# quenotl/PARESIS

Hardware: AMD Instinct MI355X
Metric: Mpixels/s, 4096^2 Fresnel+refraction step (higher is better)
Workload: dtype f32; 1 GPU; 4096x4096 fp32 study grid, 1 membrane position per GPU per step, 4 propagation distances z={1.6,3.6,5.2,7.2} m: 4 x (Fresnel propagation + refraction) from the 2-material membrane thickness maps (transmission evaluated inside the step); 52 keV, dSM/dMO/dOD=140/1.6/3.6 m; fresnel_engine=lds, streams=1, parallelism=single GPU

## Files before the change

include/paresis_hip.h:

```cpp
#ifndef PARESIS_HIP_H
#define PARESIS_HIP_H

#include <stddef.h>
#include <stdint.h>

#ifdef __cplusplus
extern "C" {
#endif

#define PSX_MAX_MAT 8
#define PSX_MAX_DIST 8
#define PSX_MAX_SRC 16

#define PSX_E_ARG (-1)
#define PSX_E_STATE (-2)
#define PSX_E_UNSUPPORTED (-3)

#define PSX_STATUS_NONFINITE 1u

typedef struct psx_fresnel_plan psx_fresnel_plan;
typedef struct psx_detector_plan psx_detector_plan;
typedef struct psx_integrate_plan psx_integrate_plan;

typedef struct { float re, im; } psx_c64;
// ... 54 lines not shown
int psx_fastloop_f32(const float *I, const float *Dx, const float *Dy, float *I2, int Nx, int Ny, void *stream);

#define PSX_ENGINE_AUTO 0
#define PSX_ENGINE_ROCFFT 1
#define PSX_ENGINE_LDS 2
int psx_fresnel_plan_create(int Nx, int Ny, int margin, int max_dist, int engine, psx_fresnel_plan **plan);
int psx_fresnel_plan_destroy(psx_fresnel_plan *plan);
int psx_fresnel_plan_engine(const psx_fresnel_plan *plan);
size_t psx_fresnel_plan_bytes(const psx_fresnel_plan *plan);
int psx_fresnel_plan_work_queue(psx_fresnel_plan *plan, int on);

int psx_fresnel_propagate(psx_fresnel_plan *plan, const psx_c64 *wave_in, float amp, const float *const *T,
                          const double *cphase, const double *catt, int nmat, int n_dist, const double *a,
                          const double *gphase, double du_x, double du_y, psx_c64 *const *wave_out,
                          float *const *inten_out, const float *inten_scale, int accumulate, void *stream);
int psx_fresnel_propagate_sources(psx_fresnel_plan *plan, int n_src, int n_dist, const psx_c64 *const *wave_in, const float *amp,
                                  const float *const *T, const double *cphase, const double *catt, int nmat, const double *a,
                                  const double *gphase, double du_x, double du_y, psx_c64 *const *wave_out,
                                  float *const *inten_out, const float *inten_scale, void *stream);

int psx_detector_plan_create(int Nx, int Ny, int ov, int nx, int ny, int margin, double sigma_src, double sigma_psf,
                             psx_detector_plan **plan);
int psx_detector_plan_destroy(psx_detector_plan *plan);
int psx_detect_f32(psx_detector_plan *plan, const float *img, float *out, void *stream);
#define PSX_MAX_DETECT 4
int psx_detect_multi_f32(psx_detector_plan *plan, const float *const *imgs, float *const *outs, int nimg, void *stream);
int psx_detector_operator_host(int N, int ov, int n, int margin, double sigma_src, double sigma_psf, int *start,
                               float *weights, int wcap, int *W_out);
int psx_resize_f32(const float *img, int Nx, int Ny, float *out, int sx, int sy, void *stream);
int psx_poisson_f32(const float *lam, float *out, int64_t n, uint64_t seed, void *stream);
// ... 72 lines not shown
```

paresis_amd/_lib.py:

```python
import ctypes
import os
from ctypes import POINTER, c_char_p, c_double, c_float, c_int, c_int64, c_size_t, c_uint64, c_void_p

_HERE = os.path.dirname(os.path.abspath(__file__))
LIB_PATH = os.path.join(_HERE, "libparesis_hip.so")

PSX_MAX_MAT = 8
PSX_MAX_FOLD = 64
PSX_MAX_LCS = 64
PSX_MAX_UMPA_WINDOW = 8
PSX_MAX_UMPA_SEARCH = 8
PSX_PHANTOM_TUBES = 12
PSX_MAX_DIST = 8
PSX_MAX_POISSON = 8
PSX_MAX_DETECT = 4
PSX_MAX_SRC = 16
PSX_SUM_SLOTS, PSX_SUM_STRIDE = 32, 16
ENGINE_AUTO, ENGINE_ROCFFT, ENGINE_LDS = 0, 1, 2
STATUS_NONFINITE = 1
ABI_VERSION = 14


class PsxError(RuntimeError):
    pass


_vp = c_void_p
_dp = POINTER(c_double)
_fp = POINTER(c_float)
_vpp = POINTER(c_void_p)

PROTOTYPES = {
    "psx_abi_version": (c_int, []),
    "psx_last_error": (c_char_p, []),
    "psx_device_ok": (c_int, []),
# ... 13 lines not shown
    "psx_refract_f32": (c_int, [_vp, c_float, _vpp, _dp, _dp, c_int, _vp, _vp, c_float, c_int, _vp, _vp, _vp, c_int,
                                c_int, c_int, c_double, c_double, c_double, _vp, _vp, _vp]),
    "psx_refract_split_f32": (c_int, [_vp, _vp, c_float, _vpp, _dp, _dp, c_int, _vp, _vp, _vp, c_float, c_int, c_int, c_int,
                                      c_int, c_double, c_double, c_double, _vp, _vp, _vp]),
    "psx_refract_multi_workspace_bytes": (c_size_t, [c_int, c_int, c_int]),
    "psx_refract_multi_f32": (c_int, [_vp, c_float, _vpp, _dp, _dp, c_int, _vp, _vpp, c_float, c_int, _vp, _vp, _vp,
                                      c_int, c_int, c_int, _dp, c_int, c_double, c_double, _vp, _vp, _vp]),
    "psx_refract_batch_workspace_bytes": (c_size_t, [c_int, c_int, c_int]),
    "psx_refract_batch_f32": (c_int, [c_int, _vpp, _fp, _vpp, _dp, _dp, c_int, _vpp, c_float, c_int, c_int, c_int, c_int, _dp,
                                      c_double, c_double, _vp, _vp, _vp]),
    "psx_fastloop_f32": (c_int, [_vp, _vp, _vp, _vp, c_int, c_int, _vp]),
    "psx_fresnel_plan_create": (c_int, [c_int, c_int, c_int, c_int, c_int, _vpp]),
    "psx_fresnel_plan_destroy": (c_int, [_vp]),
    "psx_fresnel_plan_engine": (c_int, [_vp]),
    "psx_fresnel_plan_bytes": (c_size_t, [_vp]),
    "psx_fresnel_plan_work_queue": (c_int, [_vp, c_int]),
    "psx_fresnel_propagate": (c_int, [_vp, _vp, c_float, _vpp, _dp, _dp, c_int, c_int, _dp, _dp, c_double, c_double,
                                      _vpp, _vpp, _fp, c_int, _vp]),
    "psx_fresnel_propagate_sources": (c_int, [_vp, c_int, c_int, _vpp, _fp, _vpp, _dp, _dp, c_int, _dp, _dp, c_double, c_double,
                                              _vpp, _vpp, _fp, _vp]),
    "psx_detector_plan_create": (c_int, [c_int, c_int, c_int, c_int, c_int, c_int, c_double, c_double, _vpp]),
    "psx_detector_plan_destroy": (c_int, [_vp]),
    "psx_detect_f32": (c_int, [_vp, _vp, _vp, _vp]),
    "psx_detect_multi_f32": (c_int, [_vp, _vpp, _vpp, c_int, _vp]),
    "psx_detector_operator_host": (c_int, [c_int, c_int, c_int, c_int, c_double, c_double, POINTER(c_int), _fp, c_int,
                                           POINTER(c_int)]),
    "psx_resize_f32": (c_int, [_vp, c_int, c_int, _vp, c_int, c_int, _vp]),
    "psx_poisson_f32": (c_int, [_vp, _vp, c_int64, c_uint64, _vp]),
    "psx_poisson_multi_f32": (c_int, [_vpp, POINTER(c_uint64), c_int, c_int64, _vp]),
    "psx_pack_counts_u16": (c_int, [_vp, _vp, c_int64, c_int64, _vp, _vp, c_int, _vp, _vp]),
# ... 62 lines not shown
```

paresis_amd/csrc/common.hpp:

```cpp
#pragma once
#include <hip/hip_runtime.h>

#include <atomic>
#include <cmath>
#include <cstdarg>
#include <cstdint>
#include <cstdio>
#include <memory>

#include "paresis_hip.h"

namespace psx {

char *err_buf();
int fail(int code, const char *fmt, ...);

#define PSX_HIP(expr)                                                                              \
    do {                                                                                           \
        hipError_t e__ = (expr);                                                                   \
        if (e__ != hipSuccess)                                                                     \
            return psx::fail((int)e__, "%s:%d: %s -> %s", __FILE__, __LINE__, #expr, hipGetErrorString(e__)); \
    } while (0)

#define PSX_REQUIRE(cond, ...)                         \
// ... 104 lines not shown
        case 0: { constexpr int NM = 0; __VA_ARGS__; } break; \
        case 1: { constexpr int NM = 1; __VA_ARGS__; } break; \
        case 2: { constexpr int NM = 2; __VA_ARGS__; } break; \
        case 3: { constexpr int NM = 3; __VA_ARGS__; } break; \
        case 4: { constexpr int NM = 4; __VA_ARGS__; } break; \
        default: { constexpr int NM = 8; __VA_ARGS__; } break; \
    }

extern unsigned long long *g_stamps;

enum DebugSwitch {
    DBG_STAMP_PASS1 = 0,
    DBG_STAMP_ROUND,
    DBG_DETECT_4PASS,
    DBG_NO_P2,
    DBG_COUNT
};
int debug_switch(DebugSwitch s);

bool prof_enabled();
int prof_begin(const char *name, hipStream_t st);
void prof_end(int handle, hipStream_t st);

struct ProfScope {
    int h;
    hipStream_t st;
    ProfScope(const char *name, hipStream_t s) : h(prof_enabled() ? prof_begin(name, s) : -1), st(s) {}
    ~ProfScope() {
        if (h >= 0) prof_end(h, st);
    }
// ... 32 lines not shown
```

paresis_amd/csrc/core.hip:

```cpp
#include <cstring>
#include <string>
#include <vector>

#include "common.hpp"

namespace psx {

char *err_buf() {
    static thread_local char buf[512] = "";
    return buf;
}

int fail(int code, const char *fmt, ...) {
    va_list ap;
    va_start(ap, fmt);
    vsnprintf(err_buf(), 512, fmt, ap);
    va_end(ap);
    return code;
}

int pack_mats(Mats &m, const float *const *T, const double *cphase, const double *catt, int nmat) {
    if (nmat < 0 || nmat > PSX_MAX_MAT) return fail(PSX_E_ARG, "nmat=%d outside [0,%d]", nmat, PSX_MAX_MAT);
    if (nmat > 0 && T == nullptr) return fail(PSX_E_ARG, "T is null with nmat=%d", nmat);
    m.n = nmat;
// ... 25 lines not shown
hipEvent_t take_event() {
    if (!g_pool.empty()) {
        hipEvent_t e = g_pool.back();
        g_pool.pop_back();
        return e;
    }
    hipEvent_t e = nullptr;
    (void)hipEventCreate(&e);
    return e;
}
}

unsigned long long *g_stamps = nullptr;

namespace {
const char *const g_dbg_names[DBG_COUNT] = {"stamp_pass1", "stamp_round", "detect_4pass", "no_p2"};
const int g_dbg_default[DBG_COUNT] = {0, 1, 0, 0};
std::atomic<int> g_dbg[DBG_COUNT] = {{0}, {1}, {0}, {0}};
}

int debug_switch(DebugSwitch s) { return g_dbg[s].load(std::memory_order_relaxed); }

bool prof_enabled() { return g_prof_on; }

int prof_begin(const char *name, hipStream_t st) {
    int id = -1;
    for (size_t i = 0; i < g_names.size(); ++i)
        if (g_names[i] == name) id = (int)i;
    if (id < 0) {
        g_names.push_back(name);
        id = (int)g_names.size() - 1;
    }
    ProfRec r{take_event(), take_event(), id};
// ... 13 lines not shown
    float acc = seed + threadIdx.x;
    while (wall_clock64() - r0 < ticks) {
#pragma unroll
        for (int i = 0; i < 64; ++i) acc = fmaf(acc, 1.0000001f, 0.5f);
    }
    const unsigned long long c1 = clock64(), r1 = wall_clock64();
    if (blockIdx.x == 0 && threadIdx.x == 0) {
        out[0] = c1 - c0;
        out[1] = r1 - r0;
    }
    if (acc == 12345.678f) out[2] = 1ull;
}

extern "C" {

int psx_abi_version(void) { return 14; }

const char *psx_last_error(void) { return psx::err_buf(); }

int psx_device_ok(void) {
    psx::DevBuf<int> d;
    int h = 0;
    if (d.alloc(1)) {
        psx::fail(1, "hipMalloc failed: no usable HIP device");
        return 0;
    }
    (void)hipMemset(d.get(), 0, sizeof(int));
    psx_probe_kernel<<<1, 1>>>(d.get());
    hipError_t e = hipGetLastError();
    if (e == hipSuccess) e = hipMemcpy(&h, d.get(), sizeof(int), hipMemcpyDeviceToHost);
    if (e != hipSuccess || h != 950) {
// ... 85 lines not shown
```

paresis_amd/csrc/fresnel.hip:

```cpp
#include "fresnel_plan.hpp"

using namespace psx;

namespace {

template <int NM>
__global__ __launch_bounds__(256) void k_pad_transmit(const float2 *__restrict__ wave_in, float amp, Mats m,
                                                      float2 *__restrict__ out, int Nx, int Ny, int margin, int Px,
                                                      int Py) {
    const int64_t n = (int64_t)Px * Py;
    for (int64_t q = (int64_t)blockIdx.x * blockDim.x + threadIdx.x; q < n; q += (int64_t)gridDim.x * blockDim.x) {
        const int pi = (int)(q / Py), pj = (int)(q - (int64_t)pi * Py);
        const int i = reflect_index(pi - margin, Nx), j = reflect_index(pj - margin, Ny);
        out[q] = source_wave<NM>(wave_in, amp, m, (int64_t)i * Ny + j);
    }
}

__global__ void k_chirp_table(float2 *table, int P, double a, double du, double sre, double sim) {
    const int i = blockIdx.x * blockDim.x + threadIdx.x;
    if (i >= P) return;
    const int f = (i < (P + 1) / 2) ? i : i - P;
    const double u = (double)f * du;
    const double ph = -a * u * u;
    const double r = ph - PSX_TWO_PI * rint(ph * PSX_INV_TWO_PI);
// ... 126 lines not shown
int psx_fresnel_plan_destroy(psx_fresnel_plan *p) {
    delete p;
    return 0;
}

int psx_fresnel_plan_engine(const psx_fresnel_plan *p) { return p ? p->engine : PSX_E_ARG; }

size_t psx_fresnel_plan_bytes(const psx_fresnel_plan *p) { return p ? p->bytes : 0; }

int psx_fresnel_plan_work_queue(psx_fresnel_plan *p, int on) {
    PSX_REQUIRE(p != nullptr, "psx_fresnel_plan_work_queue: null plan");
    if (p->engine == PSX_ENGINE_LDS) lds_engine_work_queue(p, on);
    return 0;
}

int psx_fresnel_propagate(psx_fresnel_plan *plan, const psx_c64 *wave_in, float amp, const float *const *T,
                          const double *cphase, const double *catt, int nmat, int n_dist, const double *a,
                          const double *gphase, double du_x, double du_y, psx_c64 *const *wave_out,
                          float *const *inten_out, const float *inten_scale, int accumulate, void *stream) {
    PSX_REQUIRE(plan != nullptr, "psx_fresnel_propagate: null plan");
    PSX_REQUIRE(n_dist >= 1 && n_dist <= plan->max_dist, "psx_fresnel_propagate: n_dist=%d outside [1,%d]", n_dist,
                plan->max_dist);
    PSX_REQUIRE(a != nullptr, "psx_fresnel_propagate: null distance table");
    PSX_REQUIRE(wave_out || inten_out, "psx_fresnel_propagate: no output requested");
    for (int d = 0; d < n_dist; ++d) {
        const bool w = wave_out && wave_out[d], i = inten_out && inten_out[d];
        PSX_REQUIRE(w || i, "psx_fresnel_propagate: distance %d has no output", d);
        PSX_REQUIRE(std::isfinite(a[d]), "psx_fresnel_propagate: a[%d] is not finite", d);
    }
    PropArgs pa;
// ... 36 lines not shown
```

paresis_amd/csrc/fresnel_lds.hip:

```cpp
#include <algorithm>
#include <cstdint>
#include <cstdlib>
#include <map>
#include <tuple>
#include <vector>

#include "fresnel_p2.hpp"
#include "fresnel_plan.hpp"
#include "fresnel_stages.hpp"

using namespace psx;
using namespace psx::lines;

namespace {

#define PSX_STAMP(k) PSX_STAMP_IF(k, tid == 0)
template <int R3, bool CONTIG, bool DUAL = false, bool QUEUE = false>
__global__ __launch_bounds__(T) void k_fresnel_lines(LineArgs a) {
    using GE = LineGeom<R3, false>;
    constexpr int M = GE::M, LINES = GE::LINES, S1 = GE::S1, MP = GE::MP;
    constexpr int LH = DUAL ? LINES / 2 : LINES;
    constexpr int LPG = LH;
    constexpr int LL = LH;
    static_assert(!DUAL || (CONTIG && LINES % 2 == 0), "DUAL: LINES/2 image lines x two distances per round");
// ... 1478 lines not shown
            }
            break;
        case Kind::P2: return p2::launch(t.radix, contig, dual, la, st, name);
        case Kind::P2X: return p2::x_launch(contig, la, st, name);
        case Kind::DIF: return contig ? launch_part<true, true>(la, st, name) : launch_part<false, true>(la, st, name);
        case Kind::PAIR: return contig ? launch_part<true, false>(la, st, name) : launch_part<false, false>(la, st, name);
    }
    return fail(PSX_E_UNSUPPORTED, "LDS engine: unsupported line length");
}

static int line_groups(const AxisTables &t, int nlines, bool dual) {
    const int lpg = t.kind == Kind::P2 ? p2::lines_per_round(t.radix, dual) : TOT / t.M / (dual ? 2 : 1);
    return (nlines + lpg - 1) / lpg;
}

static LineArgs pass_args(const psx_fresnel_plan *p, int pass, int n_dist) {
    const LdsEngine *e = p->lds.get();
    const AxisTables &t = e->ax[pass];
    LineArgs la;
    if (pass == 0) {
        la.N = p->Nx; la.nlines = p->Ny; la.P = p->Px;
        la.in_si = 1; la.in_sl = p->Nx; la.in_blocked = 0; la.out_ld = 0; la.out_blocked = 1;
    } else {
        la.N = p->Ny; la.nlines = p->Nx; la.P = p->Py;
        la.in_si = 0; la.in_sl = 0; la.in_blocked = 1; la.out_ld = p->Ny; la.out_blocked = 0;
    }
    la.margin = p->margin; la.L = la.N + la.P - 1;
    la.twA = t.twA.get(); la.twB = t.twB.get();
    la.B = t.B; la.Lh = t.Lh; la.S = t.S; la.NB = t.NB;
    la.w2 = t.w2.get(); la.w4 = t.w4.get(); la.wgpart = e->wgpart.get(); la.wg_groups = e->wgpart_groups;
    la.dsh = 2 * PART_M - la.P; la.thr = la.L - 2 * PART_M;
    la.queue = e->use_queue ? e->queue.get() + (size_t)pass * QUEUE_WORDS : nullptr;
    la.n_dist = n_dist; la.dist_inner = 0; la.accumulate = 0;
    la.stamps = nullptr; la.stamp_j = 1;
    return la;
}

int lds_engine_propagate(psx_fresnel_plan *p, const PropArgs &a) {
    LdsEngine *e = p->lds.get();
    hipStream_t st = a.stream;
    const int64_t npix = (int64_t)p->Nx * p->Ny;
    int nz[PSX_MAX_DIST], nnz = 0;
    for (int d = 0; d < a.n_dist; ++d) {
        if (a.a[d] != 0.0) {
            nz[nnz++] = d;
            continue;
        }
        PSX_DISPATCH_NMAT(a.m.n, PSX_TIMED("k_source_out", st, k_source_out<NM><<<ew_grid(npix, 256), 256, 0, st>>>(
                                                                   a.wave_in, a.amp, a.m, a.wave_out ? a.wave_out[d] : nullptr,
                                                                   a.inten_out ? a.inten_out[d] : nullptr,
                                                                   a.inten_scale ? a.inten_scale[d] : 1.f, a.accumulate,
                                                                   npix)));
    }
    if (nnz == 0) return launch_check("k_source_out");

    {
        const int ntiles = (int)(cdiv(p->Nx, 64) * cdiv(p->Ny, 64));
        int vec_ok = p->Ny % 4 == 0 && (uintptr_t)a.wave_in % 16 == 0;
        for (int i = 0; i < a.m.n && i < PSX_MAX_MAT; ++i) vec_ok = vec_ok && ((uintptr_t)a.m.T[i] % 16 == 0);
        PSX_DISPATCH_NMAT(a.m.n, PSX_TIMED("k_source_transposed", st, k_source_transposed<NM><<<ntiles, 256, 0, st>>>(
                                                                           a.wave_in, a.amp, a.m, e->pre.get(), p->Nx, p->Ny, vec_ok)));
        if (int rc = launch_check("k_source_transposed")) return rc;
    }

    const bool stamp_pass1 = debug_switch(DBG_STAMP_PASS1) != 0;
    const int stamp_round = debug_switch(DBG_STAMP_ROUND);
    {
        const AxisTables &t = e->ax[0];
        LineArgs la = pass_args(p, 0, nnz);
        la.stamps = stamp_pass1 ? g_stamps : nullptr; la.stamp_j = stamp_round;
        for (int i = 0; i < PSX_MAX_DIST; ++i) {
            const int k = i < nnz ? i : 0;
            la.src[i] = e->pre.get();
            if (i < nnz) {
                if (int rc = kernel_spectrum(p, e->ax[0], a.a[nz[i]], a.du_x, st, &la.H[i])) return rc;
            } else {
                la.H[i] = la.H[0];
            }
            la.wave_out[i] = e->inter.get() + (size_t)k * e->inter_elems;
            la.part[i] = la.wave_out[i];
            la.inten_out[i] = nullptr;
            la.scale[i] = 1.f;
            la.gph[i] = make_float2(1.f, 0.f);
        }
        const int cus = current_cu_count();
        switch (t.kind) {
            case Kind::R3:
            case Kind::P2: la.dist_inner = line_groups(t, p->Ny, nnz >= 2) >= cus; break;
            case Kind::DIF: la.dist_inner = nnz >= 2 && p->Ny >= cus; break;
            case Kind::P2X: la.dist_inner = p->Ny >= cus; break;
            case Kind::PAIR: break;
        }
        const bool dual = one_transform(t.kind) && la.dist_inner && nnz >= 2;
        if (dual && (nnz & 1)) {
            la.H[nnz] = la.H[nnz - 1];
            la.wave_out[nnz] = nullptr;
        }
        if (int rc = launch_axis(t, true, dual, la, st, "k_fresnel_cols")) return rc;
    }

    LineArgs lb = pass_args(p, 1, nnz);
    lb.accumulate = a.accumulate; lb.stamps = stamp_pass1 ? nullptr : g_stamps; lb.stamp_j = stamp_round;
    for (int i = 0; i < PSX_MAX_DIST; ++i) {
        const int k = i < nnz ? i : 0, d = nz[k];
        lb.src[i] = e->inter.get() + (size_t)k * e->inter_elems;
        if (i < nnz) {
            if (int rc = kernel_spectrum(p, e->ax[1], a.a[d], a.du_y, st, &lb.H[i])) return rc;
        } else {
            lb.H[i] = lb.H[0];
        }
        lb.wave_out[i] = a.wave_out ? a.wave_out[d] : nullptr;
        lb.part[i] = lb.wave_out[i] ? lb.wave_out[i] : (e->part ? e->part.get() + (size_t)k * npix : nullptr);
        lb.inten_out[i] = a.inten_out ? a.inten_out[d] : nullptr;
// ... 86 lines not shown
```

paresis_amd/csrc/fresnel_p2.hip:

```cpp
#include "fresnel_p2.hpp"

#include <atomic>

#include "fresnel_p2_dev.hpp"

using namespace psx;
using namespace psx::lines;
using namespace psx::p2dev;

namespace {

constexpr int TE = 512;
constexpr int TLD = 256;
constexpr int TT = TE + TLD;
constexpr int TOT2 = 16384;
constexpr int LXM = psx::p2::LXMAX;

template <int R1_, bool DUAL_>
struct G2 {
    static constexpr int R1 = R1_, M = 256 * R1, LINES = TOT2 / M, LH = DUAL_ ? LINES / 2 : LINES;
    static constexpr int MP = M + M / 32 + LXM;
    static constexpr int NBA = 32 / R1;
    static constexpr int SPL = M / 16;
    static constexpr int LB = R1 == 32 ? 5 : (R1 == 16 ? 4 : (R1 == 8 ? 3 : 2));
    static constexpr int LDP = LB | 1, LDB = 17;
    static constexpr int TPL = TLD / LINES, NCH = TPL >= 2 * LXM ? TPL / LXM : 1, CL = LXM / NCH;
    static constexpr int O_TP = LINES * MP, O_TB = O_TP + 256 * LDP, O_SA = O_TB + 16 * LDB, O_C = O_SA + LH * LXM,
                         O_UQ = O_C + NCH * LINES * LXM, O_HT = O_UQ + 2;
    static constexpr size_t lds_bytes(int ntap) { return sizeof(float2) * (size_t)(O_HT + ntap * LXM); }
    static constexpr int max_taps = (160 * 1024 / (int)sizeof(float2) - O_HT) / LXM < MAX_LINE ? (160 * 1024 / (int)sizeof(float2) - O_HT) / LXM : MAX_LINE;
    static_assert(LINES >= 2 && NBA >= 1 && max_taps >= 16, "LDS budget");
};

#define PSX_STAMP(k) PSX_STAMP_IF(k, tid == 0)

template <int R1, bool CONTIG, bool DUAL, bool QUEUE>
__global__ __launch_bounds__(TT) void k_fresnel_p2(LineArgs a) {
    using GE = G2<R1, DUAL>;
    constexpr int M = GE::M, LINES = GE::LINES, LH = GE::LH, MP = GE::MP, NBA = GE::NBA, SPL = GE::SPL, LDP = GE::LDP, LDB = GE::LDB;
    constexpr int NCH = GE::NCH, CL = GE::CL, TPL = GE::TPL;
    constexpr int LPG = LH;
    constexpr int LL = LH;
    static_assert(!DUAL || CONTIG, "DUAL is pass 1");
    extern __shared__ __attribute__((aligned(16))) float2 lds[];
    v2f *const Lb = reinterpret_cast<v2f *>(lds);
    v2f *const tP = Lb + GE::O_TP, *const tB = Lb + GE::O_TB;
    v2f *const SA = Lb + GE::O_SA;
    v2f *const CF = Lb + GE::O_C;
    v2f *const HT = Lb + GE::O_HT;
    int *const uq = reinterpret_cast<int *>(Lb + GE::O_UQ);
    const int tid = threadIdx.x;
    const int N = a.N, mg = a.margin;
    const int Lx = a.L - M;
    const bool upper_half = ((a.P - 1) >> 8) >= R1 / 2;

    const int ngroups = (a.nlines + LPG - 1) / LPG;
    const int nwork = a.dist_inner ? ngroups : ngroups * a.n_dist;
    const int xcd = blockIdx.x & 7, slot = blockIdx.x >> 3, nslot = gridDim.x >> 3;
    const int cq = nwork >> 3, cr = nwork & 7;
    const int cstart = xcd * cq + (xcd < cr ? xcd : cr), clen = cq + (xcd < cr ? 1 : 0);
    const int nunits = slot < clen ? (clen - slot + nslot - 1) / nslot : 0;
    const int nsub = DUAL ? (a.n_dist + 1) / 2 : a.n_dist;
    const int nj = a.dist_inner ? nunits * nsub : nunits;
    constexpr bool DYN = QUEUE;
    const int nsubr = a.dist_inner ? nsub : 1;
    auto item = [&](int j, int &d, int &g) __attribute__((always_inline)) {
        if (a.dist_inner) {
            const int u = j / nsub;
            d = j - u * nsub;
            g = cstart + (DYN ? uq[u & 3] : slot + u * nslot);
        } else {
            const int wk = cstart + (DYN ? uq[j & 3] : slot + j * nslot);
            d = wk / ngroups;
            g = wk - d * ngroups;
        }
    };
    auto valid = [&](int j) __attribute__((always_inline)) { return DYN ? uq[(j / nsubr) & 3] >= 0 : j < nj; };
    auto qcount = [&](int v) __attribute__((always_inline)) { return &a.queue[16 * (xcd + 8 * v)]; };
    auto share = [&](int v) __attribute__((always_inline)) { return v < clen ? (clen - v + nslot - 1) / nslot : 0; };
    bool dry = false, own_dry = false;
// ... 63 lines not shown
        const int ja = i0 + N + 2 * mg - 1, jb = i0 - 1;
        const int oa = phys(ja), ob = phys(jb);
        float2 *sa_line = lds + GE::O_SA + line * LXM;

        constexpr int CH = LL / 2 > 0 ? LL / 2 : 1, STEPV = TLD / CH, NLV = M / (2 * STEPV), PSTEPV = STEPV + STEPV / 32;
        static_assert(CONTIG || (LL % 2 == 0 && IB % 2 == 0 && STEPV % 32 == 0 && NLV * STEPV == M / 2), "16-byte loads of the blocked intermediate");
        const int c2 = lt % CH, i0v = lt / CH;
        float2 *base_v = lds + 2 * c2 * MP;
        const int jav = i0v + N + 2 * mg - 1, jbv = i0v - 1;
        const int oav = phys(jav), obv = phys(jbv);
        float2 *sa_v = lds + GE::O_SA + 2 * c2 * LXM;
        const int voff_v = ((((2 * c2) / IB) * N + i0v) * IB + (2 * c2) % IB) * (int)sizeof(float2);

        float2 xs[CONTIG ? NLD : 1], xm = make_float2(0.f, 0.f);
        float4 xv[CONTIG ? 1 : NLV];
        auto fetch = [&](int j) __attribute__((always_inline)) {
            int d, g;
            item(j, d, g);
            if (a.dist_inner && d != 0) return;
            const float2 *src = a.src[d];
            const int l0 = g * LPG;
            if constexpr (!CONTIG) {
                constexpr int LLB = LL > IB ? LL / IB : 1;
                const int nblk = min(LLB, (a.nlines - l0 + IB - 1) / IB);
                const __amdgpu_buffer_rsrc_t rs = __builtin_amdgcn_make_buffer_rsrc(
                    const_cast<float2 *>(src) + ((int64_t)(l0 / IB) * N) * IB + l0 % IB, 0,
                    nblk * N * IB * (int)sizeof(float2) - (l0 % IB) * (int)sizeof(float2), 0x00020000);
#pragma unroll
                for (int k = 0; k < NLV; ++k) {
                    const v4u r = __builtin_amdgcn_raw_buffer_load_b128(rs, voff_v + k * (STEPV * IB * (int)sizeof(float2)), 0, 0);
// ... 59 lines not shown
                    } else {
                        base[phys(ja + STEP * k)] = x;
                        if (k > 0 || jb >= 0) base[phys(jb + STEP * k)] = x;
                    }
                    if (STEP * k <= LXM) {
                        const int js = jb + STEP * k;
                        if ((unsigned)js < (unsigned)LXM) sa_line[js] = x;
                    }
                }
            }
            if (im >= 0) lds[lm * MP + phys(jm)] = l0 + lm < a.nlines ? xm : make_float2(0.f, 0.f);
            for (int t = lt + TLD; t < nmir; t += TLD) {
                const int ln = t % LL, r = t / LL;
                const int i2 = r < mg ? r + 1 : N - 1 - 2 * mg + r, j2 = r < mg ? N + 2 * mg - 1 - i2 : 2 * N - 3 - i2;
                float2 x2 = make_float2(0.f, 0.f);
                if (l0 + ln < a.nlines)
                    x2 = a.src[d][a.in_blocked ? ((int64_t)((l0 + ln) / IB) * N + i2) * IB + (l0 + ln) % IB
                                            : (int64_t)i2 * a.in_si + (int64_t)(l0 + ln) * a.in_sl];
                lds[ln * MP + phys(j2)] = x2;
            }
        };
        auto fixup = [&](int j) __attribute__((always_inline)) {
            if (Lx <= 0) return;
            int d, g;
            item(j, d, g);
            int lo = lt;
            asm volatile("" : "+v"(lo));
            const int lb = lo / TPL, r = lo % TPL;
            const int lbi = DUAL ? lb % LH : lb;
            const int dd = DUAL ? 2 * d + lb / LH : d;
            const v2f *ht = HT + dd * LXM;
            const v2f *sa = SA + lbi * LXM;
            const v2f *sb = Lb + lbi * MP + M + M / 32;
// ... 1 lines not shown
            for (int mp = NCH > 1 ? r % LXM : r; mp < LXM; mp += (NCH > 1 ? LXM : TPL)) {
                v2f acc = (v2f){0.f, 0.f};
#pragma unroll
                for (int tt = 0; tt < CL; ++tt) {
                    const int t = c * CL + tt;
                    const int jx = mp >= t ? mp - t : 0;
                    const v2f dl = lds_read(sb + jx) - lds_read(sa + jx);
                    const v2f term = pk_cmul(dl, lds_read(ht + t));
                    acc += mp >= t ? term : (v2f){0.f, 0.f};
                }
                CF[(c * LINES + lb) * LXM + mp] = acc;
            }
        };

        if (valid(0)) {
            fetch(0);
            spread(0);
        }
        lds_barrier();
        int ucur = 0, usub = 0;
        auto ring_ok = [&](int u) __attribute__((always_inline)) { return uq[u & 3] >= 0; };
        for (int j = 0; DYN ? ring_ok(ucur) : j < nj; ++j) {
            const bool last_sub = usub + 1 == nsubr;
            const bool more = DYN ? ring_ok(last_sub ? ucur + 1 : ucur) : j + 1 < nj;
            lds_barrier();
            if (a.stamps && lt == 0 && j == a.stamp_j) a.stamps[(size_t)blockIdx.x * 32 + 16] = wall_clock64();
            const bool qround = DYN && lt < 64 && usub == 0;
            const bool claiming = qround && ring_ok(ucur + 1);
            unsigned mine = 0xffffffffu;
            if (claiming && !own_dry && lt == 0) mine = atomicAdd(qcount(slot), 1u);
            if (more) fetch(j + 1);
            if (a.stamps && lt == 0 && j == a.stamp_j) a.stamps[(size_t)blockIdx.x * 32 + 17] = wall_clock64();
            fixup(j);
            lds_barrier();
            lds_barrier();
            if (a.stamps && lt == 0 && j == a.stamp_j) a.stamps[(size_t)blockIdx.x * 32 + 18] = wall_clock64();
            __builtin_amdgcn_s_setprio(3);
            if (more) spread(j + 1);
            __builtin_amdgcn_s_setprio(0);
            if (qround) {
                int unit = -1;
                if (claiming) {
                    const unsigned k = __builtin_amdgcn_readfirstlane(mine);
                    if (k < (unsigned)myshare) unit = slot + (int)k * nslot;
                    else own_dry = true;
                    if (unit < 0 && !dry) unit = steal();
                }
                if (lt == 0) uq[(ucur + 2) & 3] = unit;
// ... 223 lines not shown
                const int welems = lok ? (a.out_blocked ? ((N + IB - 1) / IB) * IB * a.nlines : N) : 0;
                if (upper_half)
                    store_legs<R1, R1 / 2>(v[i], v[i][0] + cf[i], wo, io, wbase, welems, e0, estep, (v2f){a.gph[dd].x, a.gph[dd].y},
                                           a.scale[dd], a.accumulate);
                else
                    store_legs<R1, 0>(v[i], v[i][0] + cf[i], wo, io, wbase, welems, e0, estep, (v2f){a.gph[dd].x, a.gph[dd].y},
                                      a.scale[dd], a.accumulate);
            }
        }
        PSX_STAMP(12);
        lds_barrier();
        PSX_STAMP(13);
    }
}

__global__ void k_p2_twiddles(float2 *twA, float2 *twB, int R1, int LB) {
    const int idx = blockIdx.x * blockDim.x + threadIdx.x;
    const int M = 256 * R1;
    if (idx < 256 * LB) {
        const int n = idx / LB, b = idx % LB;
        double s, c;
        sincospi(-2.0 * (double)((n << b) % M) / (double)M, &s, &c);
        twA[idx] = make_float2((float)c, (float)s);
    }
    if (idx < 256) {
        const int n = idx >> 4, k = idx & 15;
        double s, c;
        sincospi(-2.0 * (double)((n * k) % 256) / 256.0, &s, &c);
        twB[idx] = make_float2((float)c, (float)s);
    }
// ... 1 lines not shown

__global__ void k_p2_perm(const double2 *__restrict__ Hh, const double2 *__restrict__ hP, float2 *__restrict__ out, int R1, int P) {
    const int p = blockIdx.x * blockDim.x + threadIdx.x;
    const int M = 256 * R1;
    if (p < M) {
        const int k1 = p >> 8, k2 = (p >> 4) & 15, k3 = p & 15;
        const double2 v = Hh[k1 + R1 * k2 + 16 * R1 * k3];
        out[p] = make_float2((float)(v.x / M), (float)(v.y / M));
    } else if (p < M + LXM) {
        const int t = p - M;
        const double2 v = t < P ? hP[t] : make_double2(0.0, 0.0);
        out[p] = make_float2((float)(v.x / P), (float)(v.y / P));
    }
}

int line_grid_slots(int nwork, int cap) {
    int nslot = current_cu_count() / 8;
    if (nslot > (nwork + 7) / 8) nslot = (nwork + 7) / 8;
    if (cap && nslot > cap) nslot = cap;
    return nslot;
}

template <int R1, bool CONTIG, bool DUAL, bool QUEUE = false>
int launch_t(const LineArgs &la, hipStream_t st, const char *name) {
    if constexpr (!QUEUE) {
        if (la.queue) return launch_t<R1, CONTIG, DUAL, true>(la, st, name);
    }
    using GE = G2<R1, DUAL>;
    static std::atomic<unsigned long long> attr_mask{0};
    if (first_on_device(attr_mask))
        PSX_HIP(hipFuncSetAttribute((const void *)k_fresnel_p2<R1, CONTIG, DUAL, QUEUE>, hipFuncAttributeMaxDynamicSharedMemorySize,
                                    (int)GE::lds_bytes(GE::max_taps)));
    if (la.n_dist < 1 || la.n_dist > MAX_LINE || (DUAL && !la.dist_inner))
        return fail(PSX_E_STATE, "LDS engine (power-of-two lines): %d distances, dist_inner %d", la.n_dist, la.dist_inner);
    const int ntap = DUAL ? 2 * ((la.n_dist + 1) / 2) : la.n_dist;
    if (ntap > GE::max_taps) return fail(PSX_E_STATE, "LDS engine (power-of-two lines): %d distances in one launch, %d fit", ntap, GE::max_taps);
    const int nwork = ((la.nlines + GE::LH - 1) / GE::LH) * (la.dist_inner ? 1 : la.n_dist);
    const int nslot = line_grid_slots(nwork, QUEUE ? 32 : 0);
    PSX_TIMED(name, st, k_fresnel_p2<R1, CONTIG, DUAL, QUEUE><<<8 * nslot, TT, GE::lds_bytes(ntap), st>>>(la));
    const int rc = launch_check(name);
    if constexpr (QUEUE) {
        if (rc) (void)hipMemsetAsync(la.queue, 0, sizeof(unsigned) * QUEUE_WORDS, st);
    }
    return rc;
}

template <int R1>
int launch_r(bool contig, bool dual, const LineArgs &la, hipStream_t st, const char *name) {
    if (dual) return launch_t<R1, true, true>(la, st, name);
    return contig ? launch_t<R1, true, false>(la, st, name) : launch_t<R1, false, false>(la, st, name);
}

}

namespace psx {
namespace p2 {

int pick_r1(int N, int margin) {
    const int P = N + 2 * margin, L = N + P - 1;
    for (int r1 : {4, 8, 16, 32}) {
        const int M = 256 * r1;
        if (N <= M / 2 && P <= M && L - M <= LXMAX && L - M <= N - 1) return r1;
    }
    return 0;
}

static int log2_r1(int R1) { return R1 == 32 ? 5 : (R1 == 16 ? 4 : (R1 == 8 ? 3 : 2)); }
size_t twA_elems(int R1) { return (size_t)256 * log2_r1(R1); }
int max_distances(int R1) {
    switch (R1) {
        case 4: return G2<4, false>::max_taps;
// ... 15 lines not shown
    const int n = 256 * R1 + LXMAX;
    PSX_TIMED("k_kern_perm", st, k_p2_perm<<<(n + 255) / 256, 256, 0, st>>>(Hh, hP, out, R1, P));
    return launch_check("k_p2_perm");
}

int launch(int R1, bool contig, bool dual, const lines::LineArgs &la, hipStream_t st, const char *name) {
    switch (R1) {
        case 4: return launch_r<4>(contig, dual, la, st, name);
        case 8: return launch_r<8>(contig, dual, la, st, name);
        case 16: return launch_r<16>(contig, dual, la, st, name);
        case 32: return launch_r<32>(contig, dual, la, st, name);
    }
    return fail(PSX_E_UNSUPPORTED, "LDS engine (power-of-two lines): unsupported radix %d", R1);
}

}
}
```

paresis_amd/csrc/fresnel_p2.hpp:

```cpp
#pragma once
#include "fresnel_stages.hpp"

namespace psx {
namespace p2 {

constexpr int LXMAX = 32;

int pick_r1(int N, int margin);

size_t twA_elems(int R1);
size_t twB_elems();
int build_tables(float2 *twA, float2 *twB, int R1, hipStream_t st);

size_t spectrum_elems(int R1);
int perm_spectrum(const double2 *Hh, const double2 *hP, float2 *out, int R1, int P, hipStream_t st);

int launch(int R1, bool contig, bool dual, const lines::LineArgs &la, hipStream_t st, const char *name);

int max_distances(int R1);

int lines_per_round(int R1, bool dual);

bool x_serves(int N, int margin);
int x_points();
size_t x_spectrum_elems();
size_t x_line_buffer_elems();
int x_build_twiddles(float2 *w2, float2 *w4, hipStream_t st);
int x_pad_taps(const double2 *hP, double2 *buf, int P, hipStream_t st);
int x_perm_spectrum(const double2 *Hh, const double2 *hP, float2 *out, int P, hipStream_t st);
int x_launch(bool contig, const lines::LineArgs &la, hipStream_t st, const char *name);

}
}
// ... 1 lines not shown
```

paresis_amd/csrc/fresnel_plan.hpp:

```cpp
#pragma once
#include <rocfft/rocfft.h>

#include "common.hpp"

#define PSX_ROCFFT(expr)                                                                          \
    do {                                                                                          \
        rocfft_status s__ = (expr);                                                               \
        if (s__ != rocfft_status_success)                                                         \
            return psx::fail(1000 + (int)s__, "%s:%d: %s -> rocfft_status %d", __FILE__, __LINE__, #expr, (int)s__); \
    } while (0)

namespace psx {

int rocfft_ensure_setup();

class FftPlan {
    rocfft_plan plan_[2] = {nullptr, nullptr};
    rocfft_execution_info info_ = nullptr;
    DevBuf<char> work_;

  public:
    enum Dir { FWD = 0, INV = 1, BOTH = 2 };
    FftPlan() = default;
    FftPlan(const FftPlan &) = delete;
// ... 97 lines not shown
    pa.du_x = a.du_x; pa.du_y = a.du_y;
    pa.wave_out = a.wave_out ? a.wave_out + (size_t)s * a.n_dist : nullptr;
    pa.inten_out = a.inten_out ? a.inten_out + (size_t)s * a.n_dist : nullptr;
    pa.inten_scale = a.inten_scale ? a.inten_scale + (size_t)s * a.n_dist : nullptr;
    pa.accumulate = 0; pa.stream = a.stream;
    return pa;
}

int rocfft_engine_create(psx_fresnel_plan *p);
int rocfft_engine_propagate(psx_fresnel_plan *p, const PropArgs &a);

bool lds_engine_supported(int Nx, int Ny, int margin);
int lds_engine_create(psx_fresnel_plan *p);
int lds_engine_propagate(psx_fresnel_plan *p, const PropArgs &a);
void lds_engine_work_queue(psx_fresnel_plan *p, int on);
int lds_engine_propagate_sources(psx_fresnel_plan *p, const SourcesArgs &a);

template <int NM>
__device__ __forceinline__ float2 source_wave(const float2 *__restrict__ wave_in, float amp, const Mats &m, int64_t p) {
    float2 w = wave_in ? wave_in[p] : make_float2(1.f, 0.f);
    float a = amp;
    if (NM > 0) {
        double ph, la;
        mats_eval<NM>(m, p, ph, la);
        float c, s;
        cis_f64(ph, c, s);
        a *= exp_att(la);
        w = make_float2(w.x * c - w.y * s, w.x * s + w.y * c);
    }
    return make_float2(a * w.x, a * w.y);
}

__host__ __device__ __forceinline__ int reflect_index(int q, int n) {
    if (q < 0) q = -q;
    if (q >= n) q = 2 * (n - 1) - q;
    return q;
}

}
```

paresis_amd/csrc/fresnel_stages.hpp:

```cpp
#pragma once
#include <cstdint>
#include <type_traits>

#include "fft_pk.hpp"
#include "common.hpp"

namespace psx {
namespace lines {

typedef unsigned v2u __attribute__((ext_vector_type(2)));
typedef unsigned v4u __attribute__((ext_vector_type(4)));

constexpr int TC = 768;
constexpr int TL = 256;
constexpr int T = TC + TL;
constexpr int TOT = 18432;
constexpr int RAD = 24;
constexpr int IB = 8;
constexpr int IBS = 3;
static_assert((1 << IBS) == IB, "intermediate block size");
constexpr int SAMPLE_SHIFT = 3;
constexpr int BLOCKED_SAMPLE_SHIFT = IBS + SAMPLE_SHIFT;
static_assert((1 << SAMPLE_SHIFT) == sizeof(float2) && (1 << BLOCKED_SAMPLE_SHIFT) == IB * sizeof(float2),
              "sample strides of the intermediate");
// ... 16 lines not shown
    int out_blocked;
    const float2 *twA, *twB;
    const float2 *H[MAX_LINE];
    float2 *wave_out[MAX_LINE];
    float *inten_out[MAX_LINE];
    float scale[MAX_LINE];
    float2 gph[MAX_LINE];
    int accumulate;
    int B, Lh, S, NB;
    float2 *part[MAX_LINE];
    const float2 *w2;
    const float2 *w4;
    float2 *wgpart;
    int wg_groups;
    int dsh, thr;
    unsigned *queue;
    unsigned long long *stamps;
    int stamp_j;
};

#define PSX_STAMP_IF(k, who)                                                                       \
    do {                                                                                           \
        if (a.stamps && j == a.stamp_j && (who)) a.stamps[(size_t)blockIdx.x * 32 + (k)] = wall_clock64(); \
    } while (0)

__device__ __forceinline__ void wave_sync() {
    __builtin_amdgcn_fence(__ATOMIC_RELEASE, "wavefront");
    __builtin_amdgcn_wave_barrier();
    __builtin_amdgcn_fence(__ATOMIC_ACQUIRE, "wavefront");
}
// ... 204 lines not shown
```

Baseline: 62530 Mpixel/s.

## Fuse source-wave evaluation from thickness maps into the first LDS Fresnel pass

Adds a fused-source variant of the power-of-two LDS column kernel. It reads the material thickness maps directly through buffer loads and evaluates the transmitted wave in registers, instead of first writing a precomputed source field to an intermediate buffer and reading it back. This removes one full-grid complex write and read per step. The cost is extra register pressure and double-precision cis/exp work inside the FFT kernel, along with more template instantiations and a separate translation unit. It is gated on radix, map count, no wave input and no work queue, and can be disabled with a debug switch.

Result: slower. 54840 Mpixel/s (-12.3%).

```diff
diff --git a/include/paresis_hip.h b/include/paresis_hip.h
--- a/include/paresis_hip.h
+++ b/include/paresis_hip.h
@@ -92,6 +92,7 @@
                           const double *cphase, const double *catt, int nmat, int n_dist, const double *a,
                           const double *gphase, double du_x, double du_y, psx_c64 *const *wave_out,
                           float *const *inten_out, const float *inten_scale, int accumulate, void *stream);
+int psx_fresnel_fused_source(int Nx, int Ny, int margin, int n_dist, int nmat, int has_wave_in);
 int psx_fresnel_propagate_sources(psx_fresnel_plan *plan, int n_src, int n_dist, const psx_c64 *const *wave_in, const float *amp,
                                   const float *const *T, const double *cphase, const double *catt, int nmat, const double *a,
                                   const double *gphase, double du_x, double du_y, psx_c64 *const *wave_out,
diff --git a/paresis_amd/_lib.py b/paresis_amd/_lib.py
--- a/paresis_amd/_lib.py
+++ b/paresis_amd/_lib.py
@@ -18,7 +18,7 @@
 PSX_SUM_SLOTS, PSX_SUM_STRIDE = 32, 16
 ENGINE_AUTO, ENGINE_ROCFFT, ENGINE_LDS = 0, 1, 2
 STATUS_NONFINITE = 1
-ABI_VERSION = 14
+ABI_VERSION = 15
 
 
 class PsxError(RuntimeError):
@@ -62,6 +62,7 @@
     "psx_fresnel_plan_destroy": (c_int, [_vp]),
     "psx_fresnel_plan_engine": (c_int, [_vp]),
     "psx_fresnel_plan_bytes": (c_size_t, [_vp]),
+    "psx_fresnel_fused_source": (c_int, [c_int, c_int, c_int, c_int, c_int, c_int]),
     "psx_fresnel_plan_work_queue": (c_int, [_vp, c_int]),
     "psx_fresnel_propagate": (c_int, [_vp, _vp, c_float, _vpp, _dp, _dp, c_int, c_int, _dp, _dp, c_double, c_double,
                                       _vpp, _vpp, _fp, c_int, _vp]),
diff --git a/paresis_amd/csrc/common.hpp b/paresis_amd/csrc/common.hpp
--- a/paresis_amd/csrc/common.hpp
+++ b/paresis_amd/csrc/common.hpp
@@ -142,6 +142,7 @@
     DBG_STAMP_ROUND,
     DBG_DETECT_4PASS,
     DBG_NO_P2,
+    DBG_NO_FUSED_SOURCE,
     DBG_COUNT
 };
 int debug_switch(DebugSwitch s);
diff --git a/paresis_amd/csrc/core.hip b/paresis_amd/csrc/core.hip
--- a/paresis_amd/csrc/core.hip
+++ b/paresis_amd/csrc/core.hip
@@ -63,9 +63,9 @@
 unsigned long long *g_stamps = nullptr;
 
 namespace {
-const char *const g_dbg_names[DBG_COUNT] = {"stamp_pass1", "stamp_round", "detect_4pass", "no_p2"};
-const int g_dbg_default[DBG_COUNT] = {0, 1, 0, 0};
-std::atomic<int> g_dbg[DBG_COUNT] = {{0}, {1}, {0}, {0}};
+const char *const g_dbg_names[DBG_COUNT] = {"stamp_pass1", "stamp_round", "detect_4pass", "no_p2", "no_fused_source"};
+const int g_dbg_default[DBG_COUNT] = {0, 1, 0, 0, 0};
+std::atomic<int> g_dbg[DBG_COUNT] = {{0}, {1}, {0}, {0}, {0}};
 }
 
 int debug_switch(DebugSwitch s) { return g_dbg[s].load(std::memory_order_relaxed); }
@@ -109,7 +109,7 @@
 
 extern "C" {
 
-int psx_abi_version(void) { return 14; }
+int psx_abi_version(void) { return 15; }
 
 const char *psx_last_error(void) { return psx::err_buf(); }
 
diff --git a/paresis_amd/csrc/fresnel.hip b/paresis_amd/csrc/fresnel.hip
--- a/paresis_amd/csrc/fresnel.hip
+++ b/paresis_amd/csrc/fresnel.hip
@@ -164,6 +164,12 @@
     return 0;
 }
 
+int psx_fresnel_fused_source(int Nx, int Ny, int margin, int n_dist, int nmat, int has_wave_in) {
+    PSX_REQUIRE(Nx >= 2 && Ny >= 2 && margin >= 0 && margin < Nx && margin < Ny, "psx_fresnel_fused_source: grid %dx%d, margin %d", Nx, Ny, margin);
+    PSX_REQUIRE(n_dist >= 0 && n_dist <= PSX_MAX_DIST && nmat >= 0, "psx_fresnel_fused_source: %d distances, %d maps", n_dist, nmat);
+    return lds_engine_fused_source(Nx, Ny, margin, n_dist, nmat, has_wave_in != 0) ? 1 : 0;
+}
+
 int psx_fresnel_propagate(psx_fresnel_plan *plan, const psx_c64 *wave_in, float amp, const float *const *T,
                           const double *cphase, const double *catt, int nmat, int n_dist, const double *a,
                           const double *gphase, double du_x, double du_y, psx_c64 *const *wave_out,
diff --git a/paresis_amd/csrc/fresnel_lds.hip b/paresis_amd/csrc/fresnel_lds.hip
--- a/paresis_amd/csrc/fresnel_lds.hip
+++ b/paresis_amd/csrc/fresnel_lds.hip
@@ -1516,6 +1516,16 @@
     return (nlines + lpg - 1) / lpg;
 }
 
+static bool fused_source_rule(const AxisKind &t, int Nx, int Ny, int nnz, int nmat, bool wave_in, bool queue) {
+    if (t.kind != Kind::P2 || nnz < 1) return false;
+    return p2::fused_source_serves(t.radix, Nx, Ny, nmat, wave_in, queue);
+}
+
+bool lds_engine_fused_source(int Nx, int Ny, int margin, int n_dist, int nmat, bool wave_in) {
+    if (!lds_engine_supported(Nx, Ny, margin)) return false;
+    return fused_source_rule(choose(Nx, margin), Nx, Ny, n_dist, nmat, wave_in, false);
+}
+
 static LineArgs pass_args(const psx_fresnel_plan *p, int pass, int n_dist) {
     const LdsEngine *e = p->lds.get();
     const AxisTables &t = e->ax[pass];
@@ -1534,6 +1544,7 @@
     la.dsh = 2 * PART_M - la.P; la.thr = la.L - 2 * PART_M;
     la.queue = e->use_queue ? e->queue.get() + (size_t)pass * QUEUE_WORDS : nullptr;
     la.n_dist = n_dist; la.dist_inner = 0; la.accumulate = 0;
+    la.mats = Mats{}; la.amp = 0.f; la.src_ny = 0;
     la.stamps = nullptr; la.stamp_j = 1;
     return la;
 }
@@ -1556,7 +1567,9 @@
     }
     if (nnz == 0) return launch_check("k_source_out");
 
-    {
+    const bool fused = debug_switch(DBG_NO_FUSED_SOURCE) == 0 &&
+                       fused_source_rule(e->ax[0], p->Nx, p->Ny, nnz, a.m.n, a.wave_in != nullptr, e->use_queue);
+    if (!fused) {
         const int ntiles = (int)(cdiv(p->Nx, 64) * cdiv(p->Ny, 64));
         int vec_ok = p->Ny % 4 == 0 && (uintptr_t)a.wave_in % 16 == 0;
         for (int i = 0; i < a.m.n && i < PSX_MAX_MAT; ++i) vec_ok = vec_ok && ((uintptr_t)a.m.T[i] % 16 == 0);
@@ -1573,7 +1586,7 @@
         la.stamps = stamp_pass1 ? g_stamps : nullptr; la.stamp_j = stamp_round;
         for (int i = 0; i < PSX_MAX_DIST; ++i) {
             const int k = i < nnz ? i : 0;
-            la.src[i] = e->pre.get();
+            la.src[i] = fused ? nullptr : e->pre.get();
             if (i < nnz) {
                 if (int rc = kernel_spectrum(p, e->ax[0], a.a[nz[i]], a.du_x, st, &la.H[i])) return rc;
             } else {
@@ -1598,7 +1611,14 @@
             la.H[nnz] = la.H[nnz - 1];
             la.wave_out[nnz] = nullptr;
         }
-        if (int rc = launch_axis(t, true, dual, la, st, "k_fresnel_cols")) return rc;
+        if (fused) {
+            la.mats = a.m; la.amp = a.amp; la.src_ny = p->Ny;
+            if (la.L - t.M > p2::LXMAX || la.N != t.N)
+                return fail(PSX_E_UNSUPPORTED, "LDS engine: a line of %d samples (%d points) on an axis built for %d", la.N, la.L, t.N);
+            if (int rc = p2::launch_fused(t.radix, dual, la, st, "k_fresnel_cols")) return rc;
+        } else if (int rc = launch_axis(t, true, dual, la, st, "k_fresnel_cols")) {
+            return rc;
+        }
     }
 
     LineArgs lb = pass_args(p, 1, nnz);
diff --git a/paresis_amd/csrc/fresnel_p2.hip b/paresis_amd/csrc/fresnel_p2.hip
--- a/paresis_amd/csrc/fresnel_p2.hip
+++ b/paresis_amd/csrc/fresnel_p2.hip
@@ -3,6 +3,11 @@
 #include <atomic>
 
 #include "fresnel_p2_dev.hpp"
+#include "fresnel_plan.hpp"
+
+#ifndef PSX_P2_FUSED_TU
+#define PSX_P2_FUSED_TU 0
+#endif
 
 using namespace psx;
 using namespace psx::lines;
@@ -34,8 +39,10 @@
 
 #define PSX_STAMP(k) PSX_STAMP_IF(k, tid == 0)
 
-template <int R1, bool CONTIG, bool DUAL, bool QUEUE>
+template <int R1, bool CONTIG, bool DUAL, bool QUEUE, int SRC = 0>
 __global__ __launch_bounds__(TT) void k_fresnel_p2(LineArgs a) {
+    static_assert(SRC == 0 || (CONTIG && !QUEUE && SRC <= (R1 == 4 ? 3 : 4)), "fused source: pass 1, static shares, at most four maps (R1 = 4: three)");
+    constexpr bool FUSED = SRC > 0;
     using GE = G2<R1, DUAL>;
     constexpr int M = GE::M, LINES = GE::LINES, LH = GE::LH, MP = GE::MP, NBA = GE::NBA, SPL = GE::SPL, LDP = GE::LDP, LDB = GE::LDB;
     constexpr int NCH = GE::NCH, CL = GE::CL, TPL = GE::TPL;
@@ -63,7 +70,8 @@
     const int nsub = DUAL ? (a.n_dist + 1) / 2 : a.n_dist;
     const int nj = a.dist_inner ? nunits * nsub : nunits;
     constexpr bool DYN = QUEUE;
-    const int nsubr = a.dist_inner ? nsub : 1;
+    constexpr bool FUSED1 = FUSED && !DUAL;
+    const int nsubr = FUSED1 ? 1 : (a.dist_inner ? nsub : 1);
     auto item = [&](int j, int &d, int &g) __attribute__((always_inline)) {
         if (a.dist_inner) {
             const int u = j / nsub;
@@ -157,6 +165,51 @@
 
         float2 xs[CONTIG ? NLD : 1], xm = make_float2(0.f, 0.f);
         float4 xv[CONTIG ? 1 : NLV];
+        constexpr int NM = FUSED ? SRC : 1;
+        constexpr int NPART = FUSED && !DUAL && NM * NLD > 96 ? 2 : 1, KPART = NLD / NPART;
+        float tr[FUSED ? KPART : 1][NM], tm[NM];
+        using KAll = std::integral_constant<int, FUSED ? NLD : 0>;
+        using KNone = std::integral_constant<int, 0>;
+        auto gather = [&](int j, auto k0c, auto k1c) __attribute__((always_inline)) {
+            constexpr int K0 = decltype(k0c)::value, K1 = decltype(k1c)::value;
+            int d, g;
+            item(j, d, g);
+            const int l0 = g * LPG;
+            const int voff = (i0 * a.src_ny + l0 + line) * (int)sizeof(float), vstep = STEP * a.src_ny * (int)sizeof(float);
+            const int voffm = (im >= 0 && l0 + lm < a.nlines) ? (im * a.src_ny + l0 + lm) * (int)sizeof(float) : 0;
+            __amdgpu_buffer_rsrc_t rs[NM];
+#pragma unroll
+            for (int m = 0; m < NM; ++m)
+                rs[m] = __builtin_amdgcn_make_buffer_rsrc(const_cast<float *>(a.mats.T[m]), 0, N * a.src_ny * (int)sizeof(float), 0x00020000);
+#pragma unroll
+            for (int k = K0; k < K1; ++k) {
+#pragma unroll
+                for (int m = 0; m < NM; ++m)
+                    tr[k - K0][m] = __builtin_bit_cast(float, __builtin_amdgcn_raw_buffer_load_b32(rs[m], voff + k * vstep, 0, 0));
+            }
+            if constexpr (K0 == 0) {
+#pragma unroll
+                for (int m = 0; m < NM; ++m) tm[m] = __builtin_bit_cast(float, __builtin_amdgcn_raw_buffer_load_b32(rs[m], voffm, 0, 0));
+            }
+        };
+        auto evaluate = [&](auto k0c, auto k1c) __attribute__((always_inline)) {
+            constexpr int K0 = decltype(k0c)::value, K1 = decltype(k1c)::value;
+#pragma unroll
+            for (int k = K0; k < K1; ++k) {
+                xs[k] = source_wave_maps<NM>(a.amp, a.mats, tr[k - K0]);
+                if (k % 4 == 3) __builtin_amdgcn_sched_barrier(0);
+            }
+            if constexpr (K0 == 0) xm = source_wave_maps<NM>(a.amp, a.mats, tm);
+        };
+        auto gather_evaluate = [&](int j) __attribute__((always_inline)) {
+            auto part = [&](auto pc) __attribute__((always_inline)) {
+                constexpr int K0 = decltype(pc)::value * KPART;
+                gather(j, std::integral_constant<int, K0>{}, std::integral_constant<int, K0 + KPART>{});
+                evaluate(std::integral_constant<int, K0>{}, std::integral_constant<int, K0 + KPART>{});
+            };
+            part(std::integral_constant<int, 0>{});
+            if constexpr (NPART == 2) part(std::integral_constant<int, 1>{});
+        };
         auto fetch = [&](int j) __attribute__((always_inline)) {
             int d, g;
             item(j, d, g);
@@ -246,9 +299,19 @@
                 const int ln = t % LL, r = t / LL;
                 const int i2 = r < mg ? r + 1 : N - 1 - 2 * mg + r, j2 = r < mg ? N + 2 * mg - 1 - i2 : 2 * N - 3 - i2;
                 float2 x2 = make_float2(0.f, 0.f);
-                if (l0 + ln < a.nlines)
-                    x2 = a.src[d][a.in_blocked ? ((int64_t)((l0 + ln) / IB) * N + i2) * IB + (l0 + ln) % IB
-                                            : (int64_t)i2 * a.in_si + (int64_t)(l0 + ln) * a.in_sl];
+                if (l0 + ln < a.nlines) {
+                    if constexpr (FUSED) {
+                        float t2[NM];
+#pragma unroll
+                        for (int m = 0; m < NM; ++m)
+                            t2[m] = __builtin_bit_cast(float, __builtin_amdgcn_raw_buffer_load_b32(
+                                __builtin_amdgcn_make_buffer_rsrc(const_cast<float *>(a.mats.T[m]), 0, N * a.src_ny * (int)sizeof(float), 0x00020000),
+                                (i2 * a.src_ny + l0 + ln) * (int)sizeof(float), 0, 0));
+                        x2 = source_wave_maps<NM>(a.amp, a.mats, t2);
+                    } else
+                        x2 = a.src[d][a.in_blocked ? ((int64_t)((l0 + ln) / IB) * N + i2) * IB + (l0 + ln) % IB
+                                                : (int64_t)i2 * a.in_si + (int64_t)(l0 + ln) * a.in_sl];
+                }
                 lds[ln * MP + phys(j2)] = x2;
             }
         };
@@ -280,7 +343,8 @@
         };
 
         if (valid(0)) {
-            fetch(0);
+            if constexpr (FUSED) gather_evaluate(0);
+            else fetch(0);
             spread(0);
         }
         lds_barrier();
@@ -295,9 +359,25 @@
             const bool claiming = qround && ring_ok(ucur + 1);
             unsigned mine = 0xffffffffu;
             if (claiming && !own_dry && lt == 0) mine = atomicAdd(qcount(slot), 1u);
-            if (more) fetch(j + 1);
+            if constexpr (FUSED1) {
+            } else if constexpr (FUSED) {
+                if (usub == 0 && j + nsubr < nj) gather(j + nsubr, KNone{}, KAll{});
+            } else {
+                if (more) fetch(j + 1);
+            }
             if (a.stamps && lt == 0 && j == a.stamp_j) a.stamps[(size_t)blockIdx.x * 32 + 17] = wall_clock64();
             fixup(j);
+            if constexpr (FUSED) {
+                if (a.stamps && lt == 0 && j == a.stamp_j) a.stamps[(size_t)blockIdx.x * 32 + 24] = wall_clock64();
+                if (more && last_sub) {
+                    if constexpr (FUSED1) gather_evaluate(j + 1);
+                    else evaluate(KNone{}, KAll{});
+                } else if constexpr (FUSED1) {
+#pragma unroll
+                    for (int k = 0; k < NLD; ++k) xs[k] = make_float2(0.f, 0.f);
+                }
+                if (a.stamps && lt == 0 && j == a.stamp_j) a.stamps[(size_t)blockIdx.x * 32 + 25] = wall_clock64();
+            }
             lds_barrier();
             lds_barrier();
             if (a.stamps && lt == 0 && j == a.stamp_j) a.stamps[(size_t)blockIdx.x * 32 + 18] = wall_clock64();
@@ -551,6 +631,7 @@
     }
 }
 
+#if !PSX_P2_FUSED_TU
 __global__ void k_p2_twiddles(float2 *twA, float2 *twB, int R1, int LB) {
     const int idx = blockIdx.x * blockDim.x + threadIdx.x;
     const int M = 256 * R1;
@@ -582,6 +663,8 @@
     }
 }
 
+#endif
+
 int line_grid_slots(int nwork, int cap) {
     int nslot = current_cu_count() / 8;
     if (nslot > (nwork + 7) / 8) nslot = (nwork + 7) / 8;
@@ -589,15 +672,19 @@
     return nslot;
 }
 
-template <int R1, bool CONTIG, bool DUAL, bool QUEUE = false>
+template <int R1, bool CONTIG, bool DUAL, bool QUEUE = false, int SRC = 0>
 int launch_t(const LineArgs &la, hipStream_t st, const char *name) {
-    if constexpr (!QUEUE) {
+    if constexpr (SRC > 0) {
+        if (la.queue || la.mats.n != SRC || (!DUAL && la.dist_inner && la.n_dist > 1) ||
+            !p2::fused_source_serves(R1, la.N, la.nlines, SRC, false, false))
+            return fail(PSX_E_STATE, "LDS engine (power-of-two lines): fused source with %d maps on a launch it does not serve", la.mats.n);
+    } else if constexpr (!QUEUE) {
         if (la.queue) return launch_t<R1, CONTIG, DUAL, true>(la, st, name);
     }
     using GE = G2<R1, DUAL>;
     static std::atomic<unsigned long long> attr_mask{0};
     if (first_on_device(attr_mask))
-        PSX_HIP(hipFuncSetAttribute((const void *)k_fresnel_p2<R1, CONTIG, DUAL, QUEUE>, hipFuncAttributeMaxDynamicSharedMemorySize,
+        PSX_HIP(hipFuncSetAttribute((const void *)k_fresnel_p2<R1, CONTIG, DUAL, QUEUE, SRC>, hipFuncAttributeMaxDynamicSharedMemorySize,
                                     (int)GE::lds_bytes(GE::max_taps)));
     if (la.n_dist < 1 || la.n_dist > MAX_LINE || (DUAL && !la.dist_inner))
         return fail(PSX_E_STATE, "LDS engine (power-of-two lines): %d distances, dist_inner %d", la.n_dist, la.dist_inner);
@@ -605,7 +692,7 @@
     if (ntap > GE::max_taps) return fail(PSX_E_STATE, "LDS engine (power-of-two lines): %d distances in one launch, %d fit", ntap, GE::max_taps);
     const int nwork = ((la.nlines + GE::LH - 1) / GE::LH) * (la.dist_inner ? 1 : la.n_dist);
     const int nslot = line_grid_slots(nwork, QUEUE ? 32 : 0);
-    PSX_TIMED(name, st, k_fresnel_p2<R1, CONTIG, DUAL, QUEUE><<<8 * nslot, TT, GE::lds_bytes(ntap), st>>>(la));
+    PSX_TIMED(name, st, k_fresnel_p2<R1, CONTIG, DUAL, QUEUE, SRC><<<8 * nslot, TT, GE::lds_bytes(ntap), st>>>(la));
     const int rc = launch_check(name);
     if constexpr (QUEUE) {
         if (rc) (void)hipMemsetAsync(la.queue, 0, sizeof(unsigned) * QUEUE_WORDS, st);
@@ -613,16 +700,49 @@
     return rc;
 }
 
+#if PSX_P2_FUSED_TU
+template <int R1, int NM>
+int launch_f(bool dual, const LineArgs &la, hipStream_t st, const char *name) {
+    if constexpr (NM >= 1 && NM <= (R1 == 4 ? 3 : 4))
+        return dual ? launch_t<R1, true, true, false, NM>(la, st, name) : launch_t<R1, true, false, false, NM>(la, st, name);
+    else
+        return fail(PSX_E_UNSUPPORTED, "LDS engine (power-of-two lines): no fused-source kernel for %d maps", la.mats.n);
+}
+#else
 template <int R1>
 int launch_r(bool contig, bool dual, const LineArgs &la, hipStream_t st, const char *name) {
     if (dual) return launch_t<R1, true, true>(la, st, name);
     return contig ? launch_t<R1, true, false>(la, st, name) : launch_t<R1, false, false>(la, st, name);
 }
+#endif
 
 }
 
 namespace psx {
 namespace p2 {
+
+#if PSX_P2_FUSED_TU
+
+int launch_fused(int R1, bool dual, const lines::LineArgs &la, hipStream_t st, const char *name) {
+#define PSX_P2_FUSED_R1(R)                                                   \
+    case R: PSX_DISPATCH_NMAT(la.mats.n, return launch_f<R, NM>(dual, la, st, name)); break
+    switch (R1) {
+        PSX_P2_FUSED_R1(4);
+        PSX_P2_FUSED_R1(8);
+        PSX_P2_FUSED_R1(16);
+        PSX_P2_FUSED_R1(32);
+    }
+#undef PSX_P2_FUSED_R1
+    return fail(PSX_E_UNSUPPORTED, "LDS engine (power-of-two lines): unsupported radix %d", R1);
+}
+
+#else
+
+bool fused_source_serves(int R1, int N, int nlines, int nmat, bool wave_in, bool queue) {
+    if (R1 != 4 && R1 != 8 && R1 != 16 && R1 != 32) return false;
+    if (nmat < 1 || nmat > (R1 == 4 ? 3 : 4) || wave_in || queue) return false;
+    return N <= 128 * R1 && ((int64_t)128 * R1 + 1) * nlines * (int64_t)sizeof(float) < ((int64_t)1 << 31);
+}
 
 int pick_r1(int N, int margin) {
     const int P = N + 2 * margin, L = N + P - 1;
@@ -668,5 +788,7 @@
     return fail(PSX_E_UNSUPPORTED, "LDS engine (power-of-two lines): unsupported radix %d", R1);
 }
 
-}
-}
+#endif
+
+}
+}
diff --git a/paresis_amd/csrc/fresnel_p2.hpp b/paresis_amd/csrc/fresnel_p2.hpp
--- a/paresis_amd/csrc/fresnel_p2.hpp
+++ b/paresis_amd/csrc/fresnel_p2.hpp
@@ -17,6 +17,9 @@
 
 int launch(int R1, bool contig, bool dual, const lines::LineArgs &la, hipStream_t st, const char *name);
 
+bool fused_source_serves(int R1, int N, int nlines, int nmat, bool wave_in, bool queue);
+int launch_fused(int R1, bool dual, const lines::LineArgs &la, hipStream_t st, const char *name);
+
 int max_distances(int R1);
 
 int lines_per_round(int R1, bool dual);
diff --git a/paresis_amd/csrc/fresnel_plan.hpp b/paresis_amd/csrc/fresnel_plan.hpp
--- a/paresis_amd/csrc/fresnel_plan.hpp
+++ b/paresis_amd/csrc/fresnel_plan.hpp
@@ -135,6 +135,7 @@
 int lds_engine_create(psx_fresnel_plan *p);
 int lds_engine_propagate(psx_fresnel_plan *p, const PropArgs &a);
 void lds_engine_work_queue(psx_fresnel_plan *p, int on);
+bool lds_engine_fused_source(int Nx, int Ny, int margin, int n_dist, int nmat, bool wave_in);
 int lds_engine_propagate_sources(psx_fresnel_plan *p, const SourcesArgs &a);
 
 template <int NM>
@@ -152,6 +153,22 @@
     return make_float2(a * w.x, a * w.y);
 }
 
+template <int NM>
+__device__ __forceinline__ float2 source_wave_maps(float amp, const Mats &m, const float (&t)[NM]) {
+    double ph = 0.0, la = 0.0;
+#pragma unroll
+    for (int i = 0; i < NM; ++i) {
+        ph = fma(m.cphase[i], (double)t[i], ph);
+        la = fma(m.catt[i], (double)t[i], la);
+    }
+    float2 w = make_float2(1.f, 0.f);
+    float a = amp, c, s;
+    cis_f64(ph, c, s);
+    a *= exp_att(la);
+    w = make_float2(w.x * c - w.y * s, w.x * s + w.y * c);
+    return make_float2(a * w.x, a * w.y);
+}
+
 __host__ __device__ __forceinline__ int reflect_index(int q, int n) {
     if (q < 0) q = -q;
     if (q >= n) q = 2 * (n - 1) - q;
diff --git a/paresis_amd/csrc/fresnel_stages.hpp b/paresis_amd/csrc/fresnel_stages.hpp
--- a/paresis_amd/csrc/fresnel_stages.hpp
+++ b/paresis_amd/csrc/fresnel_stages.hpp
@@ -54,6 +54,9 @@
     float2 *wgpart;
     int wg_groups;
     int dsh, thr;
+    Mats mats;
+    float amp;
+    int src_ny;
     unsigned *queue;
     unsigned long long *stamps;
     int stamp_j;
```
